# jjery2243542/semi-supervised-ASR

Measured on AMD Instinct MI355X. Metric: utterances/sec (train step), higher is better.
Workload: dtype f32 (fp32-equivalent bf16x6 products)

## Files before the change

semi-supervised-asr_amd/csrc/dec_persist.hip:

```cpp
#include "persist.h"
#if defined(ASR_DP_TRACE2)
#define DP_MARK(k) do { if (tid == 0 && g == 0 && TRS >= 8 && TRS < 16) \
    ((unsigned long long*)(a.ctrl + 16))[(slice * 8 + (TRS - 8)) * 16 + (k)] = __builtin_amdgcn_s_memrealtime(); } while (0)
#elif defined(ASR_DP_TRACE)
#define DP_MARK(k) do { if (tid == 0 && g == 0 && slice == 0 && TRS >= 8 && TRS < 16) \
    ((unsigned long long*)(a.ctrl + 16))[(TRS - 8) * 16 + (k)] = clock64(); } while (0)
#else
#define DP_MARK(k) do {} while (0)
#endif

namespace {

constexpr int DP_NT = 512;
constexpr int DP_TPM = 128;
constexpr int DP_FPC = 16;
constexpr int DP_KMAX = 100;
constexpr int DP_TAPS4 = 208;
template <int RG_, int TPM_>
struct DecGeo {
  static constexpr int RG = RG_, TPM = TPM_;
  static constexpr int PPR = 32 / RG;
  static constexpr int LR = RG == 4 ? 3 : 4;
  static constexpr int FPT = 16 / RG;
  static constexpr int NFQ = RG == 4 ? 2 : 3;
// ... 598 lines not shown
    }
    __syncthreads();
    DP_MARK(9);
    {
      float acc = 0.f;
      const int oc = o_l_ < OQ ? o_l_ : 0;
      for (int t0 = wave; t0 < Tp; t0 += 32) {
        float wv[4], qv[4];
#pragma unroll
        for (int u = 0; u < 4; ++u) {
          const int t = t0 + 8 * u < Tp ? t0 + 8 * u : t0;
          wv[u] = wsm[t];
          qv[u] = Qs[t * OQ + oc];
        }
#pragma unroll
        for (int u = 0; u < 4; ++u) acc += t0 + 8 * u < Tp ? wv[u] * qv[u] : 0.f;
      }
      cpart[wave * 64 + o_l_] = acc;
    }
    __syncthreads();
    if (ctx_thread_) {
      float v = bo_v;
#pragma unroll
      for (int w2 = 0; w2 < 8; ++w2) v += cpart[w2 * 64 + tid_];
      const int o = OQ * aq + tid_;
      const float vm = drop ? v * mask_cur : v;
      if (ab_ok) {
        a.X[((int64_t)(s + 1) * B + ab) * KX + DD + o] = v;
        if (drop && s + 1 < L) a.Xd[((int64_t)(s + 1) * B + ab) * KX + DD + o] = vm;
      }
      word_store(xg + DX_C + par * 4 * 512 + ar * 512 + o, vm, bit);
      if (FB && drop) word_store(xg + DX_U + par * 4 * 512 + ar * 512 + o, v, bit);
    }
    DP_MARK(10);
#undef TRS
  }
}

template <int DD, int AA, int OO, int EE, bool FB, int RG = 4, int TPM = DP_TPM, bool FAULT = false>
int launch_dec_fwd(const DecPersistArgs& a, hipStream_t stream) {
  using DM = DecDims<DD, AA, OO, EE, RG, TPM>;
  const size_t lds = DM::lds_floats * sizeof(float);
  static_assert(DM::lds_floats * sizeof(float) > 82 * 1024 && DM::lds_floats * sizeof(float) <= 160 * 1024, "LDS budget");
  static_assert(!FB || (EE == 128 && DD % 64 == 0 && OO % 64 == 0), "free-running feedback mapping");
  hipError_t e = hipFuncSetAttribute((const void*)dec_persist_fwd_kernel<DD, AA, OO, EE, FB, RG, TPM, FAULT>,
                                     hipFuncAttributeMaxDynamicSharedMemorySize, (int)lds);
  if (e != hipSuccess) return (int)e;
  hipLaunchKernelGGL((dec_persist_fwd_kernel<DD, AA, OO, EE, FB, RG, TPM, FAULT>), dim3(256), dim3(DP_NT), lds, stream, a);
  return 0;
}


template <int TPM>
struct BwdX {
  static constexpr int C_ = 0;
  static constexpr int W_ = C_ + 2 * 4 * 512;
  static constexpr int D_ = W_ + 2 * 4 * TPM;
  static constexpr int G_ = D_ + 2 * 4 * 512;
  static constexpr int P_ = G_ + 2 * 4 * 2048;
  static constexpr int L_ = P_ + 2 * 32 * 4 * 36;
  static constexpr int GROUP = L_ + 2 * 4 * 36;
};

struct DecPersistBwdArgs {
  int B, nb, Tp, C, K, L;
  float scaling;
  const float *Q, *wcatT, *wdecT, *convw, *watt, *gvec, *w0, *xmask;
  const float *gates, *cstate, *S, *fconv, *ws, *Mf, *dws;
  float *G, *dgates, *dD, *dP, *dgvec_part, *dwatt_part, *dconv_part;
  float* dbg;
  float* xch;
  unsigned* ctrl;
  int V;
  float fb_scale;
  const float *w_out, *emb, *probs;
  float* dlfb;
};

template <int DD, int AA, int OO>
struct DecBwdDims {
  static constexpr int GK = 4 * DD;
  static constexpr int GKW = GK / 8;
  static constexpr int GKS = GK / 16;
  static constexpr int GS = GK + 4;
  static constexpr int DU = DD / 32, AU = AA / 32, OU = OO / 32;
  static constexpr int AKW = AA / 8, AQ = AA / 32;
  static constexpr int DS = AA + 4;
  static_assert(DD % 32 == 0 && AA % 32 == 0 && OO % 32 == 0 && GKS % 4 == 0, "slice sizes");
  static_assert(DU <= 16 && AU <= 16 && OU <= 16 && DD <= 512 && OO <= 512 && AA <= 512, "mappings");
};

struct BwdLds {
  int dgs, part, qs, dcx, fs, dps, Fs, dfh, wph, des, dwr, wsl, dds, ddp, dwext, ugs, wos, total;
  int dfs_stride, taps4;
};
template <int DD, int AA, int OO, int RG = 4, int TPM = DP_TPM>
__host__ __device__ inline BwdLds bwd_lds_plan(int Tp, int C, int K, int fbV = 0) {
  using BM = DecBwdDims<DD, AA, OO>;
  const int TpP = (Tp + 3) & ~3;
  BwdLds l;
  int o = 0;
  l.taps4 = ((2 * K + 1) + 3) & ~3;
  l.dfs_stride = TpP + 2 * K + 4;
  l.dfs_stride += (13 - (l.dfs_stride & 31) + 32) & 31;
  l.dgs = o; o += RG * BM::GS;
  l.part = o; o += 8 * 64 * 5;
  l.qs = o; o += 16 * OO;
  l.dcx = o; o += OO;
  l.fs = o; o += RG * C * TpP;
  l.dps = o; o += ((TpP + 16 / RG - 1) / (16 / RG)) * 4 * 64;
  l.Fs = o; o += C * (l.taps4 + 8);
  l.dfh = o; o += C * l.dfs_stride;
  l.wph = o; o += l.dfs_stride;
  l.des = o; o += RG * TPM;
  l.dwr = o; o += RG * TPM;
  l.wsl = o; o += RG * TPM;
  l.dds = o; o += RG * BM::DS;
  l.ddp = o; o += 8 * 4 * 16;
  l.dwext = o; o += 16;
  l.ugs = o; o += 16;
  l.wos = o; o += fbV * 32;
  l.total = o + 8;
  return l;
}

template <int DD, int AA, int OO, int EE, int RG = 4, int TPM = DP_TPM, bool FB = false>
__global__ __launch_bounds__(DP_NT) void dec_persist_bwd_kernel(DecPersistBwdArgs a) {
  static_assert(!FB || EE == 128, "the feedback backward is written for E = 128");
  using BM = DecBwdDims<DD, AA, OO>;
  using GEO = DecGeo<RG, TPM>;
  using BX = BwdX<TPM>;
  constexpr int PPR = GEO::PPR, LR = GEO::LR, FPT = GEO::FPT;
  constexpr int BX_C = BX::C_, BX_W = BX::W_, BX_D = BX::D_, BX_G = BX::G_, BX_GROUP = BX::GROUP;
  constexpr int NFR = RG == 4 ? 8 : 10;
  constexpr int NMR = RG == 4 ? 2 : 5;
  constexpr int LT = RG == 4 ? 7 : 8;
  static_assert((1 << LT) == TPM && RG * TPM == DP_NT, "one thread per (row, frame) of the attention weights");
  constexpr int KX = DD + OO + EE;
  constexpr int GK = BM::GK, GKW = BM::GKW, GKS = BM::GKS, GS = BM::GS, DU = BM::DU, AU = BM::AU, OU = BM::OU;
  constexpr int AKW = BM::AKW, AQ = BM::AQ, DS = BM::DS;
  extern __shared__ __attribute__((aligned(16))) float sm[];
  const int Tp = a.Tp, C = a.C, K = a.K, B = a.B, L = a.L, nb = a.nb;
  const int TpP = (Tp + 3) & ~3;
  const BwdLds ld = bwd_lds_plan<DD, AA, OO, RG, TPM>(Tp, C, K, FB ? a.V : 0);
  constexpr int BX_P = BX::P_, BX_L = BX::L_;
  float* wos = sm + ld.wos;
  float* dgs = sm + ld.dgs;
  float* part = sm + ld.part;
  float* Qs = sm + ld.qs;
  float* dcx = sm + ld.dcx;
  float* fs = sm + ld.fs;
  float* dPs = sm + ld.dps;
  float* Fs = sm + ld.Fs;
  float* dfh = sm + ld.dfh;
  float* wph = sm + ld.wph;
  float* des = sm + ld.des;
  float* dwr = sm + ld.dwr;
  float* wsl = sm + ld.wsl;
  float* dDs = sm + ld.dds;
  float* dDp = sm + ld.ddp;
  float* dwext = sm + ld.dwext;
  float* ugs = sm + ld.ugs;
  int* role = reinterpret_cast<int*>(sm + ld.total - 8);

  const int tid = threadIdx.x, lane = tid & 63;
  const int wave = __builtin_amdgcn_readfirstlane(tid >> 6);
  int g, slice;
  take_role(a.ctrl, role, g, slice);
  if (slice < 0) return;
  const int r0 = RG * g;
  if (r0 >= nb) return;
  const int taps = 2 * K + 1, taps4 = ld.taps4, DFS = ld.dfs_stride;
  const bool drop = a.xmask != nullptr;
  float* xg = a.xch + (int64_t)g * BX_GROUP;
  const __amdgpu_buffer_rsrc_t xrs = make_xch_rsrc(a.xch);
  bool aborted = false;
  const int ar = slice >> LR, aq = slice & (PPR - 1);
  const int ab = r0 + ar;
  const bool ab_ok = ab < nb;
  const int abc = ab_ok ? ab : r0;

  float wx[GKS];
  {
    const int blk = lane >> 2, i = lane & 3, cg = blk >> 1, ks = blk & 1;
    const int cl = 4 * (cg & 3) + i;
    const bool ok = cg < 4 ? cl < DU : cl < OU;
    const int col = cg < 4 ? DU * slice + (ok ? cl : 0) : DD + OU * slice + (ok ? cl : 0);
    const float* wr = a.wcatT + (int64_t)col * GK + wave * GKW + ks * GKS;
#pragma unroll
    for (int q4 = 0; q4 < GKS / 4; ++q4) {
      const float4 v = *reinterpret_cast<const float4*>(wr + 4 * q4);
      wx[4 * q4] = ok ? v.x : 0.f; wx[4 * q4 + 1] = ok ? v.y : 0.f;
      wx[4 * q4 + 2] = ok ? v.z : 0.f; wx[4 * q4 + 3] = ok ? v.w : 0.f;
    }
  }
  float wd[AQ];
  {
    const int blk = lane >> 2, ks = blk >> 2, ug = blk & 3, ul = 4 * ug + (lane & 3);
    const bool ok = ul < DU;
    const float* wr = a.wdecT + (int64_t)(DU * slice + (ok ? ul : 0)) * AA + wave * AKW + ks * AQ;
#pragma unroll
    for (int q = 0; q < AQ; ++q) wd[q] = ok ? wr[q] : 0.f;
  }
  for (int i = tid; i < ld.total - 8; i += DP_NT) sm[i] = 0.f;
  __syncthreads();
  for (int i = tid; i < 16 * OO; i += DP_NT) {
    const int tl = i / OO, o = i - tl * OO;
    const int t = 16 * aq + tl;
    Qs[i] = a.Q[((int64_t)abc * Tp + (t < Tp ? t : Tp - 1)) * OO + o];
  }
  const int FSS = taps4 + 8;
  for (int i = tid; i < C * FSS; i += DP_NT) {
    const int ch = i / FSS, j = i - ch * FSS;
    Fs[i] = j < taps ? a.convw[ch * taps + j] : 0.f;
  }
  if (tid < 16) {
    float v = 0.f;
    if (tid < C)
      for (int aa = 0; aa < AA; ++aa) v += a.watt[(int64_t)aa * C + tid] * a.gvec[aa];
    ugs[tid] = v;
  }
  float ereg[4] = {0.f, 0.f, 0.f, 0.f};
  if (FB) {
    for (int i = tid; i < a.V * 32; i += DP_NT) {
      const int v = i >> 5, ci = i & 31;
      const bool ok = ci < 16 ? ci < DU : ci - 16 < OU;
      const int col = ci < 16 ? DU * slice + ci : DD + OU * slice + ci - 16;
      wos[i] = ok ? a.w_out[(int64_t)v * (DD + OO) + col] : 0.f;
    }
    if (tid < 144 && tid % 36 < a.V) {
#pragma unroll
      for (int e = 0; e < 4; ++e) ereg[e] = a.emb[(tid % 36) * EE + 4 * slice + e];
    }
  }
  const float gv = (lane & 15) < AU ? a.gvec[AU * slice + (lane & 15)] : 0.f;
  f32x4 acc_watt = (f32x4){0.f, 0.f, 0.f, 0.f};
  float dgl = 0.f;
  f32x4 acc_cv0 = (f32x4){0.f, 0.f, 0.f, 0.f}, acc_cv1 = (f32x4){0.f, 0.f, 0.f, 0.f};
  float dcarry = 0.f, dxz = 0.f;
  const bool pw_thread = tid < 4 * DU;
  const int punit = DU * slice + (pw_thread ? (tid >> 2) : 0);
  const int pb = r0 + (tid & 3);
  const bool pb_ok = pw_thread && (tid & 3) < RG && pb < nb;
  const int pbc = ((tid & 3) < RG && pb < nb) ? pb : r0;
  const bool cx_thread = tid >= 64 && tid < 64 + 4 * OU;
  const int cxcol = OU * slice + (cx_thread ? ((tid - 64) >> 2) : 0);

  float sreg[16];
  float freg[NFR];
  float mreg[NMR];
  float wsreg = 0.f, wpreg = 0.f, dwsreg = 0.f;
  float4 ga = make_float4(0.f, 0.f, 0.f, 0.f);
  float ct = 0.f, cp = 0.f, gz = 0.f, gc = 0.f, xm = 1.f;
  auto prefetchA = [&](int s, int zq) {
    const int tidq = tid + zq, laneq = lane + zq;
    const int q4q = laneq >> 4, alq = laneq & 15;
    const int acolq = AU * slice + (alq < AU ? alq : 0);
#pragma unroll
    for (int it = 0; it < 4; ++it) {
#pragma unroll
      for (int i = 0; i < 4; ++i) {
        const int t = FPT * (wave + 8 * it) + (4 * q4q + i) / RG;
        const int b = r0 + (4 * q4q + i) % RG;
        const float* sb = a.S + ((int64_t)s * B + (b < nb ? b : r0)) * Tp * AA;
        sreg[it * 4 + i] = sb[(t < Tp ? t : Tp - 1) * AA + acolq];
      }
    }
    const float rct = 1.0f / (float)(C * TpP), rtp = 1.0f / (float)TpP;
    const float* fb = a.fconv + (int64_t)s * B * C * Tp;
#pragma unroll
    for (int k = 0; k < NFR; ++k) {
      const int id = tidq + DP_NT * k;
      const int row = (int)(((float)id + 0.5f) * rct), rem = id - row * C * TpP;
      const int c = (int)(((float)rem + 0.5f) * rtp), t = rem - c * TpP;
      const int b = r0 + (row < RG ? row : 0);
      freg[k] = fb[((b < nb ? b : r0) * C + (row < RG ? c : 0)) * Tp + (t < Tp ? t : Tp - 1)];
// ... 95 lines not shown
      const int row = (int)(((float)tid_ + 0.5f) * (1.0f / (float)hp)), t2 = tid_ - row * hp;
      const bool ok = row < RG;
      const u64* p[1];
      u64 v[1];
      p[0] = reinterpret_cast<const u64*>(xg + BX_W + slot * 4 * TPM + (ok ? row * TPM + 2 * t2 : 0));
      poll_pairs<1, true>(p, bit, v, a.ctrl, aborted, 22u);
      if (ok) { dwr[row * TPM + 2 * t2] = pair_lo(v[0]); dwr[row * TPM + 2 * t2 + 1] = pair_hi(v[0]); }
    }
    __syncthreads();
    if (wave < RG) {
      float w[TPM / 64], dv[TPM / 64], dot = 0.f;
#pragma unroll
      for (int k = 0; k < TPM / 64; ++k) {
        const int t = lane_ + 64 * k;
        w[k] = t < Tp ? wsl[wave * TPM + t] : 0.f;
        dv[k] = t < Tp ? dwr[wave * TPM + t] : 0.f;
        dot += w[k] * dv[k];
      }
      dot = wave_sum_dpp(dot);
#pragma unroll
      for (int k = 0; k < TPM / 64; ++k)
        des[wave * TPM + lane_ + 64 * k] = r0 + wave < nb ? a.scaling * w[k] * (dv[k] - dot) : 0.f;
    }
    __syncthreads();
    DP_MARK(3);
    {
      float dDl[4] = {0.f, 0.f, 0.f, 0.f};
#pragma unroll
      for (int it = 0; it < 4; ++it) {
        const int tile = wave + 8 * it;
        if (FPT * tile < TpP) {
#pragma unroll
          for (int i = 0; i < 4; ++i) {
            const int ri = i % RG, t = FPT * tile + (4 * q4_ + i) / RG;
            const float sv = sreg[it * 4 + i];
            const float det = des[ri * TPM + t];
            const float duv = sc_ok_ ? det * gv * (1.f - sv * sv) : 0.f;
            dPs[(tile * 4 + i) * 64 + lane_] += duv;
            dDl[ri] += duv;
            dgl += sc_ok_ ? det * sv : 0.f;
            const float fb = fs[(ri * C + (a_l_ < C ? a_l_ : 0)) * TpP + ((RG == 4 || t < TpP) ? t : 0)];
            acc_watt = __builtin_amdgcn_mfma_f32_16x16x4f32(duv, a_l_ < C ? fb : 0.f, acc_watt, 0, 0, 0);
          }
        }
      }
#pragma unroll
      for (int i = 0; i < 4; ++i) {
        float v = dDl[i];
        v += __shfl_xor(v, 16, 64);
        v += __shfl_xor(v, 32, 64);
        if (q4_ == 0) dDp[(wave * 4 + i) * 16 + a_l_] = v;
      }
    }
    __syncthreads();
    if (tid_ < 64) {
      const int row = tid_ >> 4, al = tid_ & 15;
      float v = 0.f;
#pragma unroll
      for (int w2 = 0; w2 < 8; ++w2) v += dDp[(w2 * 4 + row) * 16 + al];
      const int b = r0 + row;
      if (al < AU) {
        if (row < RG && b < nb) a.dD[((int64_t)s * B + b) * AA + AU * slice + al] = v;
        word_store(xg + BX_D + (slot * 4 + row) * 512 + AU * slice + al, v, bit);
      }
    }
    DP_MARK(4);
    {
      const float rtp = 1.0f / (float)TpP;
#pragma unroll
      for (int k = 0; k < NMR; ++k) {
        const int id = tid_ + DP_NT * k;
        if (id < C * TpP) {
          const int c = (int)(((float)id + 0.5f) * rtp), t = id - c * TpP;
          if (t < Tp) dfh[c * DFS + K + t] = des[ar * TPM + t] * (ugs[c] - mreg[k]);
        }
      }
    }
    __syncthreads();
    {
      DP_MARK(10);
      const int cb = lane_ >> 2, li = lane_ & 3;
      const bool cok = cb < C;
      const int cc = cok ? cb : 0;
      {
        f32x4 acc = (f32x4){0.f, 0.f, 0.f, 0.f}, accb = (f32x4){0.f, 0.f, 0.f, 0.f};
        const float* ap = dfh + cc * DFS + 16 * aq + 4 * li + 2 * K + 4;
        const float* bp = Fs + cc * FSS + li - 4;
        const int jend = taps + 3 + 4;
        for (int j = wave; j < jend; j += 32) {
          float av[4], bv[4];
#pragma unroll
          for (int u = 0; u < 4; ++u) {
            const int jc = j + 8 * u < jend ? j + 8 * u : j;
            av[u] = ap[-jc];
            bv[u] = bp[jc];
          }
#pragma unroll
          for (int u = 0; u < 4; u += 2) {
            const int j0 = j + 8 * u, j1 = j + 8 * (u + 1);
            acc = __builtin_amdgcn_mfma_f32_4x4x1f32((cok && j0 < jend) ? av[u] : 0.f, j0 - 4 + li >= 0 ? bv[u] : 0.f, acc, 0, 0, 0);
            accb = __builtin_amdgcn_mfma_f32_4x4x1f32((cok && j1 < jend) ? av[u + 1] : 0.f, j1 - 4 + li >= 0 ? bv[u + 1] : 0.f, accb, 0, 0, 0);
          }
        }
        float* pp = part + (wave * 64 + lane_) * 5;
#pragma unroll
        for (int i = 0; i < 4; ++i) pp[i] = acc[i] + accb[i];
      }
      {
        const float* bq = dfh + cc * DFS + K - li;
        const float* a0 = wph + 16 * aq + 4 * li;
        const bool two = 16 * (aq + PPR) < taps;
        const int uend = Tp + 3;
        for (int u = wave; u < uend; u += 32) {
          float bv[4], a0v[4], a1v[4];
#pragma unroll
          for (int k = 0; k < 4; ++k) {
            const int uc = u + 8 * k < uend ? u + 8 * k : u;
            bv[k] = bq[uc];
            a0v[k] = a0[uc];
            a1v[k] = a0[two ? uc + 16 * PPR : uc];
          }
#pragma unroll
          for (int k = 0; k < 4; ++k) {
            const float b = (cok && u + 8 * k < uend) ? bv[k] : 0.f;
            acc_cv0 = __builtin_amdgcn_mfma_f32_4x4x1f32(a0v[k], b, acc_cv0, 0, 0, 0);
            acc_cv1 = __builtin_amdgcn_mfma_f32_4x4x1f32(two ? a1v[k] : 0.f, b, acc_cv1, 0, 0, 0);
          }
        }
      }
      DP_MARK(11);
      __syncthreads();
      if (tid_ < 128) {
        const int w2 = tid_ >> 4, o = tid_ & 15, i = o >> 2, jj = o & 3;
        float v = 0.f;
        for (int c = 0; c < C; ++c) v += part[(w2 * 64 + 4 * c + jj) * 5 + i];
        dDp[w2 * 16 + o] = v;
      }
      __syncthreads();
      if (tid_ < 16) {
        float v = 0.f;
#pragma unroll
        for (int w2 = 0; w2 < 8; ++w2) v += dDp[w2 * 16 + tid_];
        dwext[tid_] = 16 * aq + tid_ < Tp ? v : 0.f;
      }
      DP_MARK(12);
    }
    DP_MARK(5);
    {
      constexpr int ND = (AA + DP_NT - 1) / DP_NT;
      const unsigned dbase = (unsigned)((xg - a.xch) + BX_D + slot * 4 * 512) * 4u;
      unsigned off[ND];
      u4v v[ND];
#pragma unroll
      for (int i = 0; i < ND; ++i) {
        const int id = tid_ + DP_NT * i;
        const int row = (4 * id) / AA, c4 = 4 * id - row * AA;
        off[i] = dbase + (unsigned)((4 * id < 4 * AA) ? row * 512 + c4 : 0) * 4u;
      }
      poll_quads<ND, true>(xrs, off, bit, v, a.ctrl, aborted, 23u);
      DP_MARK(6);
#pragma unroll
      for (int i = 0; i < ND; ++i) {
        const int id = tid_ + DP_NT * i;
        const int row = (4 * id) / AA, c4 = 4 * id - row * AA;
        if (4 * id < RG * AA)
          *reinterpret_cast<float4*>(dDs + row * DS + c4) = make_float4(__uint_as_float(v[i].x), __uint_as_float(v[i].y),
                                                                       __uint_as_float(v[i].z), __uint_as_float(v[i].w));
      }
    }
    __syncthreads();
    {
      f32x4 acc = (f32x4){0.f, 0.f, 0.f, 0.f}, accb = (f32x4){0.f, 0.f, 0.f, 0.f};
      const float* dr = dDs + ((lane_ & 3) % RG) * DS + wave * AKW + (lane_ >> 4) * AQ;
#pragma unroll
      for (int q = 0; q < AQ; q += 2) {
        acc = __builtin_amdgcn_mfma_f32_4x4x1f32(wd[q], dr[q], acc, 0, 0, 0);
        if (q + 1 < AQ) accb = __builtin_amdgcn_mfma_f32_4x4x1f32(wd[q + 1], dr[q + 1], accb, 0, 0, 0);
      }
#pragma unroll
      for (int i = 0; i < 4; ++i) acc[i] += accb[i];
      float* pp = part + (wave * 64 + lane_) * 5;
#pragma unroll
      for (int i = 0; i < 4; ++i) pp[i] = acc[i];
    }
    __syncthreads();
    if (tid_ < 4 * DU) {
      const int ul = tid_ >> 2, row = tid_ & 3, ug = ul >> 2, ii = ul & 3;
      float dh = gz + dxz;
#pragma unroll
      for (int w2 = 0; w2 < 8; ++w2)
#pragma unroll
        for (int ks = 0; ks < 4; ++ks) dh += part[(w2 * 64 + 4 * (4 * ks + ug) + row) * 5 + ii];
      const float tc = asr_fast_tanh(ct);
      const float dc = dcarry + dh * ga.w * (1.f - tc * tc);
      float4 da;
      da.x = dc * ga.z * ga.x * (1.f - ga.x);
      da.y = dc * cp * ga.y * (1.f - ga.y);
      da.z = dc * ga.x * (1.f - ga.z * ga.z);
      da.w = dh * tc * ga.w * (1.f - ga.w);
      dcarry = dc * ga.y;
      if (aborted || abort_seen != 0u) da.x = __builtin_nanf("");
      const int un = DU * slice + ul, b = r0 + row;
      if (row < RG && b < nb) *reinterpret_cast<float4*>(a.dgates + ((int64_t)s * B + b) * GK + un * 4) = da;
      float* dst = xg + BX_G + (slot * 4 + row) * 2048 + un * 4;
      word_store(dst, da.x, bit); word_store(dst + 1, da.y, bit);
      word_store(dst + 2, da.z, bit); word_store(dst + 3, da.w, bit);
    }
    DP_MARK(7);
    if (s == 0) break;
    {
      constexpr int NG = (GK + DP_NT - 1) / DP_NT;
      const unsigned gbase = (unsigned)((xg - a.xch) + BX_G + slot * 4 * 2048) * 4u;
      unsigned off[NG];
      u4v v[NG];
#pragma unroll
      for (int i = 0; i < NG; ++i) {
        const int id = tid_ + DP_NT * i;
        const int row = (4 * id) / GK, c4 = 4 * id - row * GK;
        off[i] = gbase + (unsigned)((4 * id < 4 * GK) ? row * 2048 + c4 : 0) * 4u;
      }
      poll_quads<NG, true>(xrs, off, bit, v, a.ctrl, aborted, 24u);
#pragma unroll
      for (int i = 0; i < NG; ++i) {
        const int id = tid_ + DP_NT * i;
        const int row = (4 * id) / GK, c4 = 4 * id - row * GK;
        if (4 * id < RG * GK)
          *reinterpret_cast<float4*>(dgs + row * GS + c4) = make_float4(__uint_as_float(v[i].x), __uint_as_float(v[i].y),
                                                                       __uint_as_float(v[i].z), __uint_as_float(v[i].w));
      }
    }
    __syncthreads();
    float4 wfe[4];
    float fb_mask = 1.f, fb_prob = 0.f;
    if (FB) {
      const int kcg = 64 * (wave >> 2) + lane_;
      const float4* wp = reinterpret_cast<const float4*>(a.wcatT + (int64_t)(DD + OO + 4 * slice + (wave & 3)) * GK +
                                                          (16 * kcg < GK ? 16 * kcg : 0));
#pragma unroll
      for (int i = 0; i < 4; ++i) wfe[i] = wp[i];
      const int mrow = tid_ & 3, mb = r0 + mrow;
      if (drop && tid_ < 16)
        fb_mask = a.xmask[((int64_t)s * B + (mb < nb ? mb : r0)) * (OO + EE) + OO + 4 * slice + (tid_ >> 2)];
      if (slice == 0 && wave < RG) {
        const int pb2 = r0 + wave;
        fb_prob = (lane_ < a.V && pb2 < nb) ? a.probs[((int64_t)(s - 1) * B + pb2) * a.V + lane_] : 0.f;
      }
    }
    prefetchA(s - 1, zv);
    {
      f32x4 acc = (f32x4){0.f, 0.f, 0.f, 0.f}, accb = (f32x4){0.f, 0.f, 0.f, 0.f};
      DP_MARK(8);
      const float* gr = dgs + ((lane_ & 3) % RG) * GS + wave * GKW + ((lane_ >> 2) & 1) * GKS;
#pragma unroll
      for (int q4 = 0; q4 < GKS / 4; ++q4) {
        const float4 b = *reinterpret_cast<const float4*>(gr + 4 * q4);
        acc = __builtin_amdgcn_mfma_f32_4x4x1f32(wx[4 * q4], b.x, acc, 0, 0, 0);
        accb = __builtin_amdgcn_mfma_f32_4x4x1f32(wx[4 * q4 + 1], b.y, accb, 0, 0, 0);
        acc = __builtin_amdgcn_mfma_f32_4x4x1f32(wx[4 * q4 + 2], b.z, acc, 0, 0, 0);
        accb = __builtin_amdgcn_mfma_f32_4x4x1f32(wx[4 * q4 + 3], b.w, accb, 0, 0, 0);
      }
#pragma unroll
      for (int i = 0; i < 4; ++i) acc[i] += accb[i];
      float* pp = part + (wave * 64 + lane_) * 5;
#pragma unroll
      for (int i = 0; i < 4; ++i) pp[i] = acc[i];
    }
    __syncthreads();
    float vdx = 0.f, vfb = 0.f;
    if (tid_ < 128) {
      const int ci = tid_ >> 2, row = tid_ & 3, cg = ci >> 2, ii = ci & 3;
#pragma unroll
      for (int w2 = 0; w2 < 8; ++w2)
#pragma unroll
        for (int ks = 0; ks < 2; ++ks) vdx += part[(w2 * 64 + 4 * (2 * cg + ks) + row) * 5 + ii];
    }
    if (FB) {
      float* fbr = dDp;
      {
        float pr[4] = {0.f, 0.f, 0.f, 0.f};
        const int kcg = 64 * (wave >> 2) + lane_;
        const bool kok = 16 * kcg < GK;
        const float* dg = dgs + (kok ? 16 * kcg : 0);
#pragma unroll
        for (int i = 0; i < 4; ++i)
#pragma unroll
          for (int r = 0; r < 4; ++r) {
            const float4 x = *reinterpret_cast<const float4*>(dg + (r % RG) * GS + 4 * i);
            pr[r] += wfe[i].x * x.x + wfe[i].y * x.y + wfe[i].z * x.z + wfe[i].w * x.w;
          }
#pragma unroll
        for (int r = 0; r < 4; ++r) {
          const float t = wave_sum_dpp(kok ? pr[r] : 0.f);
          if (lane_ == 0) fbr[wave * 4 + r] = t;
        }
      }
      __syncthreads();
      if (tid_ < 16) {
        const int row = tid_ & 3, ec = tid_ >> 2, b = r0 + row;
        const float v = (fbr[ec * 4 + row] + fbr[(ec + 4) * 4 + row]) * fb_mask;
        if (row < RG && b < nb) a.G[((int64_t)s * B + b) * KX + DD + OO + 4 * slice + ec] = v;
        fbr[32 + row * 4 + ec] = v;
      }
      __syncthreads();
      if (tid_ < 144) {
        const int row = tid_ / 36;
        const float* dm = fbr + 32 + row * 4;
        const float pdp = dm[0] * ereg[0] + dm[1] * ereg[1] + dm[2] * ereg[2] + dm[3] * ereg[3];
        word_store(xg + BX_P + (slot * 32 + slice) * 144 + tid_, pdp, bit);
      }
      if (slice == 0) {
        constexpr int NPQ = 3;
        const unsigned pbase = (unsigned)((xg - a.xch) + BX_P + slot * 32 * 144) * 4u;
        unsigned off[NPQ];
        u4v v[NPQ];
#pragma unroll
        for (int i = 0; i < NPQ; ++i) {
          const int q = tid_ + DP_NT * i;
          off[i] = pbase + (unsigned)(q < 32 * 36 ? q : 0) * 16u;
        }
        poll_quads<NPQ, true>(xrs, off, bit, v, a.ctrl, aborted, 25u);
        static_assert(32 * 144 <= RG * BM::GS + 8 * 64 * 5, "scratch of the feedback shares");
        __syncthreads();
#pragma unroll
        for (int i = 0; i < NPQ; ++i) {
          const int q = tid_ + DP_NT * i;
          if (q < 32 * 36)
            *reinterpret_cast<float4*>(dgs + 4 * q) = make_float4(__uint_as_float(v[i].x), __uint_as_float(v[i].y),
                                                                  __uint_as_float(v[i].z), __uint_as_float(v[i].w));
        }
        __syncthreads();
        if (wave < 4) {
          float dp = 0.f;
          if (lane_ < 36) {
#pragma unroll 8
            for (int src = 0; src < 32; ++src) dp += dgs[src * 144 + wave * 36 + lane_];
          }
          const float pdot = wave_sum_dpp(fb_prob * dp);
          const float dl = a.fb_scale * fb_prob * (dp - pdot);
          const int b = r0 + wave;
          if (lane_ < a.V && wave < RG && b < nb) a.dlfb[((int64_t)(s - 1) * B + b) * a.V + lane_] = dl;
          if (lane_ < 36) word_store(xg + BX_L + slot * 144 + wave * 36 + lane_, dl, bit);
        }
      }
      {
        const unsigned lbase = (unsigned)((xg - a.xch) + BX_L + slot * 144) * 4u;
        unsigned off[1] = {lbase + (unsigned)(tid_ < 36 ? tid_ : 0) * 16u};
        u4v v[1];
        poll_quads<1, true>(xrs, off, bit, v, a.ctrl, aborted, 26u);
        if (tid_ < 36)
          *reinterpret_cast<float4*>(fbr + 64 + 4 * tid_) = make_float4(__uint_as_float(v[0].x), __uint_as_float(v[0].y),
                                                                         __uint_as_float(v[0].z), __uint_as_float(v[0].w));
      }
      __syncthreads();
      if (tid_ < 128) {
        const int ci = tid_ >> 2, row = tid_ & 3;
        const float* dl = fbr + 64 + row * 36;
        float acc = 0.f;
        for (int v = 0; v < a.V; ++v) acc += dl[v] * wos[v * 32 + ci];
        vfb = acc;
      }
    }
    if (tid_ < 128) {
      const int ci = tid_ >> 2, row = tid_ & 3;
      const float v = vdx;
      if (ci < 16) {
        dxz = v + vfb;
      } else if (ci - 16 < OU) {
        const int col = OU * slice + ci - 16, b = r0 + row;
        const float tot = gc + v * xm + vfb;
        if (row < RG && b < nb) a.G[((int64_t)s * B + b) * KX + DD + col] = tot;
        word_store(xg + BX_C + (((n + 1) & 1) * 4 + row) * 512 + col, tot, tag_bit_of_step(n + 1));
      }
    }
    DP_MARK(9);
#undef TRS
    prefetchB(s - 1, zv);
  }
  __syncthreads();
  int ze;
  asm volatile("v_mov_b32 %0, 0" : "=v"(ze));
  const int lane_e = lane + ze, a_le = lane_e & 15, q4e = lane_e >> 4;
  const bool sc_oke = a_le < AU;
  const int acole = AU * slice + (sc_oke ? a_le : 0);
#pragma unroll
  for (int it = 0; it < 4; ++it) {
    const int tile = wave + 8 * it;
    if (FPT * tile < TpP) {
#pragma unroll
      for (int i = 0; i < 4; ++i) {
        const int b = r0 + (4 * q4e + i) % RG, t = FPT * tile + (4 * q4e + i) / RG;
        if (sc_oke && b < nb && t < Tp) a.dP[((int64_t)b * Tp + t) * AA + acole] = dPs[(tile * 4 + i) * 64 + lane_e];
      }
    }
  }
  if (sc_oke) atomicAdd(a.dgvec_part + (int64_t)r0 * AA + acole, dgl);
  {
    const int c = lane & 15;
#pragma unroll
    for (int i = 0; i < 4; ++i) {
      const int al = 4 * (lane >> 4) + i;
      if (c < C && al < AU) atomicAdd(a.dwatt_part + ((int64_t)r0 * AA + AU * slice + al) * C + c, acc_watt[i]);
    }
  }
  {
    const int c = lane_e >> 2, jj = lane_e & 3;
    if (c < C && ab_ok) {
#pragma unroll
      for (int i = 0; i < 4; ++i) {
        const int j0 = 16 * aq + 4 * i + jj, j1 = j0 + 16 * PPR;
        if (j0 < taps) atomicAdd(a.dconv_part + ((int64_t)ab * C + c) * taps + j0, acc_cv0[i]);
        if (j1 < taps) atomicAdd(a.dconv_part + ((int64_t)ab * C + c) * taps + j1, acc_cv1[i]);
      }
    }
  }
}

template <int AA>
__global__ __launch_bounds__(256) void att_m_kernel(int B, int nb, int L, int Tp, int C, const float* __restrict__ S,
                                                    const float* __restrict__ watt, const float* __restrict__ gvec,
                                                    float* __restrict__ Mf) {
  __shared__ __attribute__((aligned(16))) float UG[AA * 16];
  const int tid = threadIdx.x, lane = tid & 63, wave = tid >> 6;
  for (int i0 = 0; i0 < AA * 16; i0 += 256 * 8) {
    float wv[8], gq[8];
#pragma unroll
    for (int k = 0; k < 8; ++k) {
      const int i = i0 + 256 * k + tid, aa = (i >> 4) < AA ? (i >> 4) : AA - 1, c = i & 15;
      wv[k] = watt[(int64_t)aa * C + (c < C ? c : 0)];
      gq[k] = gvec[aa];
    }
#pragma unroll
    for (int k = 0; k < 8; ++k) {
      const int i = i0 + 256 * k + tid;
      if (i < AA * 16) UG[i] = (i & 15) < C ? wv[k] * gq[k] : 0.f;
    }
  }
  __syncthreads();
  const int r = lane & 15, q = lane >> 4;
  const int ntile = (Tp + 15) / 16;
  for (int64_t item = (int64_t)blockIdx.x * 4 + wave; item < (int64_t)nb * L * ntile; item += (int64_t)gridDim.x * 4) {
    const int pair = (int)(item / ntile), tile = (int)(item - (int64_t)pair * ntile);
    const int s = pair / nb, b = pair - s * nb;
    const float* Sb = S + ((int64_t)s * B + b) * Tp * AA;
    {
      const int t = 16 * tile + r;
      const float* row = Sb + (int64_t)(t < Tp ? t : Tp - 1) * AA + 4 * q;
      f32x4 acc = (f32x4){0.f, 0.f, 0.f, 0.f}, accb = (f32x4){0.f, 0.f, 0.f, 0.f};
#pragma unroll 16
      for (int kq = 0; kq < AA / 16; ++kq) {
        const float4 sv = *reinterpret_cast<const float4*>(row + 16 * kq);
        const float* ub = UG + (16 * kq + 4 * q) * 16 + r;
        acc = __builtin_amdgcn_mfma_f32_16x16x4f32(sv.x * sv.x, ub[0], acc, 0, 0, 0);
        accb = __builtin_amdgcn_mfma_f32_16x16x4f32(sv.y * sv.y, ub[16], accb, 0, 0, 0);
        acc = __builtin_amdgcn_mfma_f32_16x16x4f32(sv.z * sv.z, ub[32], acc, 0, 0, 0);
        accb = __builtin_amdgcn_mfma_f32_16x16x4f32(sv.w * sv.w, ub[48], accb, 0, 0, 0);
      }
      if (r < C) {
#pragma unroll
        for (int i = 0; i < 4; ++i) {
          const int tt = 16 * tile + 4 * q + i;
          if (tt < Tp) Mf[(((int64_t)s * B + b) * C + r) * Tp + tt] = acc[i] + accb[i];
        }
      }
    }
  }
}

__global__ void mask_emb_kernel(int L, int B, int nb, int D, int O, int E, const float* __restrict__ xmask,
                                float* __restrict__ G) {
  const int64_t idx = (int64_t)blockIdx.x * blockDim.x + threadIdx.x;
  if (idx >= (int64_t)L * nb * E) return;
  const int e = (int)(idx % E);
  const int64_t rb = idx / E;
  const int b = (int)(rb % nb), s = (int)(rb / nb);
  G[((int64_t)s * B + b) * (D + O + E) + D + O + e] *= xmask[((int64_t)s * B + b) * (O + E) + O + e];
}

template <int DD, int AA, int OO, int EE, int RG = 4, int TPM = DP_TPM, bool FB = false>
int launch_dec_bwd(const DecPersistBwdArgs& a, hipStream_t stream) {
  const BwdLds ld = bwd_lds_plan<DD, AA, OO, RG, TPM>(a.Tp, a.C, a.K, FB ? a.V : 0);
  size_t lds = (size_t)ld.total * sizeof(float);
  if (lds > 160 * 1024) return ASR_E_SHAPE;
  if (lds <= 82 * 1024) lds = 82 * 1024 + 64;
  hipError_t e = hipFuncSetAttribute((const void*)dec_persist_bwd_kernel<DD, AA, OO, EE, RG, TPM, FB>,
                                     hipFuncAttributeMaxDynamicSharedMemorySize, (int)lds);
  if (e != hipSuccess) return (int)e;
  hipLaunchKernelGGL((dec_persist_bwd_kernel<DD, AA, OO, EE, RG, TPM, FB>), dim3(256), dim3(DP_NT), lds, stream, a);
  return 0;
}

}

// ... 178 lines not shown
```

Measured before the change: 2730.

## Remap backward decoder MFMA loops for RG=4 non-feedback path

```diff
diff --git a/semi-supervised-asr_amd/csrc/dec_persist.hip b/semi-supervised-asr_amd/csrc/dec_persist.hip
--- a/semi-supervised-asr_amd/csrc/dec_persist.hip
+++ b/semi-supervised-asr_amd/csrc/dec_persist.hip
@@ -704,11 +704,12 @@
   static constexpr int GK = 4 * DD;
   static constexpr int GKW = GK / 8;
   static constexpr int GKS = GK / 16;
+  static constexpr int GKB = GK / 64;
   static constexpr int GS = GK + 4;
   static constexpr int DU = DD / 32, AU = AA / 32, OU = OO / 32;
   static constexpr int AKW = AA / 8, AQ = AA / 32;
   static constexpr int DS = AA + 4;
-  static_assert(DD % 32 == 0 && AA % 32 == 0 && OO % 32 == 0 && GKS % 4 == 0, "slice sizes");
+  static_assert(DD % 32 == 0 && AA % 32 == 0 && OO % 32 == 0 && GKB % 4 == 0, "slice sizes");
   static_assert(DU <= 16 && AU <= 16 && OU <= 16 && DD <= 512 && OO <= 512 && AA <= 512, "mappings");
 };
 
@@ -759,8 +760,9 @@
   constexpr int LT = RG == 4 ? 7 : 8;
   static_assert((1 << LT) == TPM && RG * TPM == DP_NT, "one thread per (row, frame) of the attention weights");
   constexpr int KX = DD + OO + EE;
-  constexpr int GK = BM::GK, GKW = BM::GKW, GKS = BM::GKS, GS = BM::GS, DU = BM::DU, AU = BM::AU, OU = BM::OU;
+  constexpr int GK = BM::GK, GKW = BM::GKW, GKS = BM::GKS, GKB = BM::GKB, GS = BM::GS, DU = BM::DU, AU = BM::AU, OU = BM::OU;
   constexpr int AKW = BM::AKW, AQ = BM::AQ, DS = BM::DS;
+  constexpr bool SWEEP = !FB && RG == 4;
   extern __shared__ __attribute__((aligned(16))) float sm[];
   const int Tp = a.Tp, C = a.C, K = a.K, B = a.B, L = a.L, nb = a.nb;
   const int TpP = (Tp + 3) & ~3;
@@ -803,17 +805,37 @@
   const int abc = ab_ok ? ab : r0;
 
   float wx[GKS];
-  {
-    const int blk = lane >> 2, i = lane & 3, cg = blk >> 1, ks = blk & 1;
-    const int cl = 4 * (cg & 3) + i;
-    const bool ok = cg < 4 ? cl < DU : cl < OU;
-    const int col = cg < 4 ? DU * slice + (ok ? cl : 0) : DD + OU * slice + (ok ? cl : 0);
-    const float* wr = a.wcatT + (int64_t)col * GK + wave * GKW + ks * GKS;
-#pragma unroll
-    for (int q4 = 0; q4 < GKS / 4; ++q4) {
-      const float4 v = *reinterpret_cast<const float4*>(wr + 4 * q4);
-      wx[4 * q4] = ok ? v.x : 0.f; wx[4 * q4 + 1] = ok ? v.y : 0.f;
-      wx[4 * q4 + 2] = ok ? v.z : 0.f; wx[4 * q4 + 3] = ok ? v.w : 0.f;
+  if constexpr (SWEEP) {
+    {
+      const int blk = lane >> 2, i = lane & 3, kb = blk >> 1, cgl = blk & 1;
+#pragma unroll
+      for (int p = 0; p < 4; ++p) {
+        const int cg = 2 * p + cgl;
+        const int cl = 4 * (cg & 3) + i;
+        const bool ok = cg < 4 ? cl < DU : cl < OU;
+        const int col = cg < 4 ? DU * slice + (ok ? cl : 0) : DD + OU * slice + (ok ? cl : 0);
+        const float* wr = a.wcatT + (int64_t)col * GK + wave * GKW + 4 * kb;
+#pragma unroll
+        for (int q4 = 0; q4 < GKB / 4; ++q4) {
+          const float4 v = *reinterpret_cast<const float4*>(wr + 32 * q4);
+          float* w = wx + p * GKB + 4 * q4;
+          w[0] = ok ? v.x : 0.f; w[1] = ok ? v.y : 0.f; w[2] = ok ? v.z : 0.f; w[3] = ok ? v.w : 0.f;
+        }
+      }
+    }
+  } else {
+    {
+      const int blk = lane >> 2, i = lane & 3, cg = blk >> 1, ks = blk & 1;
+      const int cl = 4 * (cg & 3) + i;
+      const bool ok = cg < 4 ? cl < DU : cl < OU;
+      const int col = cg < 4 ? DU * slice + (ok ? cl : 0) : DD + OU * slice + (ok ? cl : 0);
+      const float* wr = a.wcatT + (int64_t)col * GK + wave * GKW + ks * GKS;
+#pragma unroll
+      for (int q4 = 0; q4 < GKS / 4; ++q4) {
+        const float4 v = *reinterpret_cast<const float4*>(wr + 4 * q4);
+        wx[4 * q4] = ok ? v.x : 0.f; wx[4 * q4 + 1] = ok ? v.y : 0.f;
+        wx[4 * q4 + 2] = ok ? v.z : 0.f; wx[4 * q4 + 3] = ok ? v.w : 0.f;
+      }
     }
   }
   float wd[AQ];
@@ -1075,56 +1097,124 @@
       const int cb = lane_ >> 2, li = lane_ & 3;
       const bool cok = cb < C;
       const int cc = cok ? cb : 0;
-      {
-        f32x4 acc = (f32x4){0.f, 0.f, 0.f, 0.f}, accb = (f32x4){0.f, 0.f, 0.f, 0.f};
-        const float* ap = dfh + cc * DFS + 16 * aq + 4 * li + 2 * K + 4;
-        const float* bp = Fs + cc * FSS + li - 4;
-        const int jend = taps + 3 + 4;
-        for (int j = wave; j < jend; j += 32) {
-          float av[4], bv[4];
-#pragma unroll
-          for (int u = 0; u < 4; ++u) {
-            const int jc = j + 8 * u < jend ? j + 8 * u : j;
-            av[u] = ap[-jc];
-            bv[u] = bp[jc];
-          }
-#pragma unroll
-          for (int u = 0; u < 4; u += 2) {
-            const int j0 = j + 8 * u, j1 = j + 8 * (u + 1);
-            acc = __builtin_amdgcn_mfma_f32_4x4x1f32((cok && j0 < jend) ? av[u] : 0.f, j0 - 4 + li >= 0 ? bv[u] : 0.f, acc, 0, 0, 0);
-            accb = __builtin_amdgcn_mfma_f32_4x4x1f32((cok && j1 < jend) ? av[u + 1] : 0.f, j1 - 4 + li >= 0 ? bv[u + 1] : 0.f, accb, 0, 0, 0);
-          }
-        }
-        float* pp = part + (wave * 64 + lane_) * 5;
-#pragma unroll
-        for (int i = 0; i < 4; ++i) pp[i] = acc[i] + accb[i];
-      }
-      {
-        const float* bq = dfh + cc * DFS + K - li;
-        const float* a0 = wph + 16 * aq + 4 * li;
-        const bool two = 16 * (aq + PPR) < taps;
-        const int uend = Tp + 3;
-        for (int u = wave; u < uend; u += 32) {
-          float bv[4], a0v[4], a1v[4];
-#pragma unroll
-          for (int k = 0; k < 4; ++k) {
-            const int uc = u + 8 * k < uend ? u + 8 * k : u;
-            bv[k] = bq[uc];
-            a0v[k] = a0[uc];
-            a1v[k] = a0[two ? uc + 16 * PPR : uc];
-          }
-#pragma unroll
-          for (int k = 0; k < 4; ++k) {
-            const float b = (cok && u + 8 * k < uend) ? bv[k] : 0.f;
-            acc_cv0 = __builtin_amdgcn_mfma_f32_4x4x1f32(a0v[k], b, acc_cv0, 0, 0, 0);
-            acc_cv1 = __builtin_amdgcn_mfma_f32_4x4x1f32(two ? a1v[k] : 0.f, b, acc_cv1, 0, 0, 0);
+      if constexpr (SWEEP) {
+        {
+          f32x4 acc = (f32x4){0.f, 0.f, 0.f, 0.f}, accb = (f32x4){0.f, 0.f, 0.f, 0.f};
+          const float* ap = dfh + cc * DFS + 16 * aq + li + 2 * K + 12;
+          const float* bp = Fs + cc * FSS + 4 * li - 12;
+          const int nr = (taps4 >> 2) + 3;
+          const int rf = wave < nr ? wave : 0;
+          float4 bn = *reinterpret_cast<const float4*>(bp + 4 * rf);
+          float an[4];
+#pragma unroll
+          for (int e = 0; e < 4; ++e) an[e] = ap[-(4 * rf + e)];
+          for (int r = wave; r < nr; r += 8) {
+            const float4 bv = bn;
+            float av[4];
+#pragma unroll
+            for (int e = 0; e < 4; ++e) av[e] = an[e];
+            const int rn = r + 8 < nr ? r + 8 : r;
+            bn = *reinterpret_cast<const float4*>(bp + 4 * rn);
+#pragma unroll
+            for (int e = 0; e < 4; ++e) an[e] = ap[-(4 * rn + e)];
+            const int tp = 4 * r - 12 + 4 * li;
+            const float b0 = (cok && tp >= 0 && tp < taps) ? bv.x : 0.f;
+            const float b1 = (cok && tp + 1 >= 0 && tp + 1 < taps) ? bv.y : 0.f;
+            const float b2 = (cok && tp + 2 >= 0 && tp + 2 < taps) ? bv.z : 0.f;
+            const float b3 = (cok && tp + 3 >= 0 && tp + 3 < taps) ? bv.w : 0.f;
+            acc = __builtin_amdgcn_mfma_f32_4x4x1f32(av[0], b0, acc, 0, 0, 0);
+            accb = __builtin_amdgcn_mfma_f32_4x4x1f32(av[1], b1, accb, 0, 0, 0);
+            acc = __builtin_amdgcn_mfma_f32_4x4x1f32(av[2], b2, acc, 0, 0, 0);
+            accb = __builtin_amdgcn_mfma_f32_4x4x1f32(av[3], b3, accb, 0, 0, 0);
+          }
+          float* pp = part + (wave * 64 + lane_) * 5;
+#pragma unroll
+          for (int i = 0; i < 4; ++i) pp[i] = acc[i] + accb[i];
+        }
+      } else {
+        {
+          f32x4 acc = (f32x4){0.f, 0.f, 0.f, 0.f}, accb = (f32x4){0.f, 0.f, 0.f, 0.f};
+          const float* ap = dfh + cc * DFS + 16 * aq + 4 * li + 2 * K + 4;
+          const float* bp = Fs + cc * FSS + li - 4;
+          const int jend = taps + 3 + 4;
+          for (int j = wave; j < jend; j += 32) {
+            float av[4], bv[4];
+#pragma unroll
+            for (int u = 0; u < 4; ++u) {
+              const int jc = j + 8 * u < jend ? j + 8 * u : j;
+              av[u] = ap[-jc];
+              bv[u] = bp[jc];
+            }
+#pragma unroll
+            for (int u = 0; u < 4; u += 2) {
+              const int j0 = j + 8 * u, j1 = j + 8 * (u + 1);
+              acc = __builtin_amdgcn_mfma_f32_4x4x1f32((cok && j0 < jend) ? av[u] : 0.f, j0 - 4 + li >= 0 ? bv[u] : 0.f, acc, 0, 0, 0);
+              accb = __builtin_amdgcn_mfma_f32_4x4x1f32((cok && j1 < jend) ? av[u + 1] : 0.f, j1 - 4 + li >= 0 ? bv[u + 1] : 0.f, accb, 0, 0, 0);
+            }
+          }
+          float* pp = part + (wave * 64 + lane_) * 5;
+#pragma unroll
+          for (int i = 0; i < 4; ++i) pp[i] = acc[i] + accb[i];
+        }
+      }
+      if constexpr (SWEEP) {
+        {
+          constexpr int NUG = TPM / 32;
+          constexpr int UCH = 4;
+          const int cn = lane_ & 15, kq = lane_ >> 4;
+          const bool cnok = cn < C;
+          const float* bq = dfh + (cnok ? cn : 0) * DFS + K + kq;
+          const float* a0 = wph + 16 * aq + cn + kq;
+          const bool two = 16 * (aq + PPR) < taps;
+#pragma unroll
+          for (int h = 0; h < NUG; h += UCH) {
+            float bv[UCH], a0v[UCH], a1v[UCH];
+#pragma unroll
+            for (int k = 0; k < UCH; ++k) {
+              const int u0 = 4 * (wave + 8 * (h + k));
+              const int uc = u0 < TpP ? u0 : 0;
+              bv[k] = bq[uc];
+              a0v[k] = a0[uc];
+              a1v[k] = a0[uc + 16 * PPR];
+            }
+#pragma unroll
+            for (int k = 0; k < UCH; ++k) {
+              if (4 * (wave + 8 * (h + k)) < TpP) {
+                const float b = cnok ? bv[k] : 0.f;
+                acc_cv0 = __builtin_amdgcn_mfma_f32_16x16x4f32(a0v[k], b, acc_cv0, 0, 0, 0);
+                acc_cv1 = __builtin_amdgcn_mfma_f32_16x16x4f32(two ? a1v[k] : 0.f, b, acc_cv1, 0, 0, 0);
+              }
+            }
+          }
+        }
+      } else {
+        {
+          const float* bq = dfh + cc * DFS + K - li;
+          const float* a0 = wph + 16 * aq + 4 * li;
+          const bool two = 16 * (aq + PPR) < taps;
+          const int uend = Tp + 3;
+          for (int u = wave; u < uend; u += 32) {
+            float bv[4], a0v[4], a1v[4];
+#pragma unroll
+            for (int k = 0; k < 4; ++k) {
+              const int uc = u + 8 * k < uend ? u + 8 * k : u;
+              bv[k] = bq[uc];
+              a0v[k] = a0[uc];
+              a1v[k] = a0[two ? uc + 16 * PPR : uc];
+            }
+#pragma unroll
+            for (int k = 0; k < 4; ++k) {
+              const float b = (cok && u + 8 * k < uend) ? bv[k] : 0.f;
+              acc_cv0 = __builtin_amdgcn_mfma_f32_4x4x1f32(a0v[k], b, acc_cv0, 0, 0, 0);
+              acc_cv1 = __builtin_amdgcn_mfma_f32_4x4x1f32(two ? a1v[k] : 0.f, b, acc_cv1, 0, 0, 0);
+            }
           }
         }
       }
       DP_MARK(11);
       __syncthreads();
       if (tid_ < 128) {
-        const int w2 = tid_ >> 4, o = tid_ & 15, i = o >> 2, jj = o & 3;
+        const int w2 = tid_ >> 4, o = tid_ & 15, i = SWEEP ? o & 3 : o >> 2, jj = SWEEP ? o >> 2 : o & 3;
         float v = 0.f;
         for (int c = 0; c < C; ++c) v += part[(w2 * 64 + 4 * c + jj) * 5 + i];
         dDp[w2 * 16 + o] = v;
@@ -1241,31 +1331,70 @@
     }
     prefetchA(s - 1, zv);
     {
-      f32x4 acc = (f32x4){0.f, 0.f, 0.f, 0.f}, accb = (f32x4){0.f, 0.f, 0.f, 0.f};
-      DP_MARK(8);
-      const float* gr = dgs + ((lane_ & 3) % RG) * GS + wave * GKW + ((lane_ >> 2) & 1) * GKS;
-#pragma unroll
-      for (int q4 = 0; q4 < GKS / 4; ++q4) {
-        const float4 b = *reinterpret_cast<const float4*>(gr + 4 * q4);
-        acc = __builtin_amdgcn_mfma_f32_4x4x1f32(wx[4 * q4], b.x, acc, 0, 0, 0);
-        accb = __builtin_amdgcn_mfma_f32_4x4x1f32(wx[4 * q4 + 1], b.y, accb, 0, 0, 0);
-        acc = __builtin_amdgcn_mfma_f32_4x4x1f32(wx[4 * q4 + 2], b.z, acc, 0, 0, 0);
-        accb = __builtin_amdgcn_mfma_f32_4x4x1f32(wx[4 * q4 + 3], b.w, accb, 0, 0, 0);
-      }
-#pragma unroll
-      for (int i = 0; i < 4; ++i) acc[i] += accb[i];
-      float* pp = part + (wave * 64 + lane_) * 5;
-#pragma unroll
-      for (int i = 0; i < 4; ++i) pp[i] = acc[i];
+      if constexpr (SWEEP) {
+        f32x4 acc[4];
+#pragma unroll
+        for (int p = 0; p < 4; ++p) acc[p] = (f32x4){0.f, 0.f, 0.f, 0.f};
+        DP_MARK(8);
+        const float* gr = dgs + ((lane_ & 3) % RG) * GS + wave * GKW + 4 * (lane_ >> 3);
+#pragma unroll
+        for (int q4 = 0; q4 < GKB / 4; ++q4) {
+          const float4 b = *reinterpret_cast<const float4*>(gr + 32 * q4);
+#pragma unroll
+          for (int p = 0; p < 4; ++p) {
+            const float* w = wx + p * GKB + 4 * q4;
+            acc[p] = __builtin_amdgcn_mfma_f32_4x4x1f32(w[0], b.x, acc[p], 0, 0, 0);
+            acc[p] = __builtin_amdgcn_mfma_f32_4x4x1f32(w[1], b.y, acc[p], 0, 0, 0);
+            acc[p] = __builtin_amdgcn_mfma_f32_4x4x1f32(w[2], b.z, acc[p], 0, 0, 0);
+            acc[p] = __builtin_amdgcn_mfma_f32_4x4x1f32(w[3], b.w, acc[p], 0, 0, 0);
+          }
+        }
+        const bool h5 = (lane_ & 32) != 0, h4 = (lane_ & 16) != 0;
+        float* pp = part + (wave * 64 + lane_) * 5;
+#pragma unroll
+        for (int i = 0; i < 4; ++i) {
+          const float k0 = (h5 ? acc[2][i] : acc[0][i]) + __shfl_xor(h5 ? acc[0][i] : acc[2][i], 32, 64);
+          const float k1 = (h5 ? acc[3][i] : acc[1][i]) + __shfl_xor(h5 ? acc[1][i] : acc[3][i], 32, 64);
+          float v = (h4 ? k1 : k0) + __shfl_xor(h4 ? k0 : k1, 16, 64);
+          v += __shfl_xor(v, 8, 64);
+          pp[i] = v;
+        }
+      } else {
+        f32x4 acc = (f32x4){0.f, 0.f, 0.f, 0.f}, accb = (f32x4){0.f, 0.f, 0.f, 0.f};
+        DP_MARK(8);
+        const float* gr = dgs + ((lane_ & 3) % RG) * GS + wave * GKW + ((lane_ >> 2) & 1) * GKS;
+#pragma unroll
+        for (int q4 = 0; q4 < GKS / 4; ++q4) {
+          const float4 b = *reinterpret_cast<const float4*>(gr + 4 * q4);
+          acc = __builtin_amdgcn_mfma_f32_4x4x1f32(wx[4 * q4], b.x, acc, 0, 0, 0);
+          accb = __builtin_amdgcn_mfma_f32_4x4x1f32(wx[4 * q4 + 1], b.y, accb, 0, 0, 0);
+          acc = __builtin_amdgcn_mfma_f32_4x4x1f32(wx[4 * q4 + 2], b.z, acc, 0, 0, 0);
+          accb = __builtin_amdgcn_mfma_f32_4x4x1f32(wx[4 * q4 + 3], b.w, accb, 0, 0, 0);
+        }
+#pragma unroll
+        for (int i = 0; i < 4; ++i) acc[i] += accb[i];
+        float* pp = part + (wave * 64 + lane_) * 5;
+#pragma unroll
+        for (int i = 0; i < 4; ++i) pp[i] = acc[i];
+      }
     }
     __syncthreads();
     float vdx = 0.f, vfb = 0.f;
-    if (tid_ < 128) {
-      const int ci = tid_ >> 2, row = tid_ & 3, cg = ci >> 2, ii = ci & 3;
-#pragma unroll
-      for (int w2 = 0; w2 < 8; ++w2)
-#pragma unroll
-        for (int ks = 0; ks < 2; ++ks) vdx += part[(w2 * 64 + 4 * (2 * cg + ks) + row) * 5 + ii];
+    if constexpr (SWEEP) {
+      if (tid_ < 128) {
+        const int ci = tid_ >> 2, row = tid_ & 3, cg = ci >> 2, ii = ci & 3;
+        const int pl = 32 * (cg >> 2) + 16 * ((cg >> 1) & 1) + 4 * (cg & 1) + row;
+#pragma unroll
+        for (int w2 = 0; w2 < 8; ++w2) vdx += part[(w2 * 64 + pl) * 5 + ii];
+      }
+    } else {
+      if (tid_ < 128) {
+        const int ci = tid_ >> 2, row = tid_ & 3, cg = ci >> 2, ii = ci & 3;
+#pragma unroll
+        for (int w2 = 0; w2 < 8; ++w2)
+#pragma unroll
+          for (int ks = 0; ks < 2; ++ks) vdx += part[(w2 * 64 + 4 * (2 * cg + ks) + row) * 5 + ii];
+      }
     }
     if (FB) {
       float* fbr = dDp;
@@ -1388,19 +1517,19 @@
   }
   if (sc_oke) atomicAdd(a.dgvec_part + (int64_t)r0 * AA + acole, dgl);
   {
-    const int c = lane & 15;
+    const int c = SWEEP ? a_le : lane & 15;
 #pragma unroll
     for (int i = 0; i < 4; ++i) {
-      const int al = 4 * (lane >> 4) + i;
+      const int al = 4 * (SWEEP ? q4e : lane >> 4) + i;
       if (c < C && al < AU) atomicAdd(a.dwatt_part + ((int64_t)r0 * AA + AU * slice + al) * C + c, acc_watt[i]);
     }
   }
   {
-    const int c = lane_e >> 2, jj = lane_e & 3;
+    const int c = SWEEP ? lane_e & 15 : lane_e >> 2, jj = SWEEP ? lane_e >> 4 : lane_e & 3;
     if (c < C && ab_ok) {
 #pragma unroll
       for (int i = 0; i < 4; ++i) {
-        const int j0 = 16 * aq + 4 * i + jj, j1 = j0 + 16 * PPR;
+        const int j0 = 16 * aq + (SWEEP ? 4 * jj + i : 4 * i + jj), j1 = j0 + 16 * PPR;
         if (j0 < taps) atomicAdd(a.dconv_part + ((int64_t)ab * C + c) * taps + j0, acc_cv0[i]);
         if (j1 < taps) atomicAdd(a.dconv_part + ((int64_t)ab * C + c) * taps + j1, acc_cv1[i]);
       }
```

Result: faster. 2767 (median of 6 runs) (+1.3%).
